# elfi-dev/elfi

Measured on AMD Instinct MI355X. Metric: ABC distances/sec, higher is better.
Workload: dtype f64; 1 GPU; configs[1]: synthetic Gaussian summaries, 1000000 samples x 32 summaries per GPU per step, elfi.Distance('euclidean'), inputs resident in HBM; samples_per_gpu=1000000, summaries=32, layout=row-major (n,m) f64, batches_in_rotation=3, exchange=none (N = 1), exchange_every=8, world_size_seen=1

## Files before the change

### elfi_amd/csrc/distance.hip

```cpp
#include "common.hpp"
#include "tile_stream.hpp"
#include "internal.hpp"
#include "np_sum.hpp"

#pragma clang fp contract(off)

namespace elfihip {

constexpr int kMaxTileM = 299;
constexpr int kMaxK = 64;

__device__ __forceinline__ double cbrt_halley(double s) {
  if (!(s > 0.0) || !(s < __builtin_huge_val())) return s;
  int e;
  double mant = frexp(s, &e);
  int q = e / 3, r = e - 3 * q;
  if (r < 0) {
    r += 3;
    q -= 1;
  }
  mant = ldexp(mant, r);
  double y = (double)__builtin_exp2f(__builtin_log2f((float)mant) * (1.0f / 3.0f));
  const double y3 = y * y * y;
  y = y * ((y3 + 2.0 * mant) / (2.0 * y3 + mant));
// ... 144 lines not shown
#pragma unroll 4
      for (int j = 0; j < m; ++j) {
        const double xc = kCentered ? x(j) - xmu : x(j);
        const double yc = kCentered ? y(j) - o.ymu : y(j);
        uv += xc * (yc * a(j));
        uu += xc * (xc * a(j));
      }
      return clip02(1.0 - uv / sqrt(uu * o.ynorm));
    } else {
      double xmu = 0.0;
      if constexpr (kCentered) xmu = np_pairwise_bounded<2>(x, 0, m) / (double)m;
      auto cx = [&](int j) { return kCentered ? x(j) - xmu : x(j); };
      auto cy = [&](int j) { return kCentered ? y(j) - o.ymu : y(j); };
      double s0 = 0.0, s1 = 0.0, q0 = 0.0, q1 = 0.0;
      int j = 0;
#pragma unroll 4
      for (; j + 1 < m; j += 2) {
        const double x0 = cx(j), x1 = cx(j + 1);
        s0 += x0 * cy(j);
        s1 += x1 * cy(j + 1);
        q0 += x0 * x0;
        q1 += x1 * x1;
      }
      double s = s0 + s1, q = q0 + q1;
      if (m & 1) {
        const double xl = cx(m - 1);
        s += xl * cy(m - 1);
        q += xl * xl;
      }
      return cos_finish(s, sqrt(q), o.ynorm);
    }
  }

  __device__ static __forceinline__ double cos_finish(double dot, double nx, double ny) {
    double c = dot / (nx * ny);
    if (fabs(c) > 1.0) c = copysign(1.0, c);
    return 1.0 - c;
  }
  __device__ static __forceinline__ double clip02(double d) { return d < 0.0 ? 0.0 : (d > 2.0 ? 2.0 : d); }

  __device__ static __forceinline__ double wide(const double* __restrict__ x, const double* __restrict__ y,
                                                const double* __restrict__ w, int m, int lane, const Obs& o) {
    auto wsum = [](double v) {
#pragma unroll
      for (int off = 32; off > 0; off >>= 1) v += __shfl_xor(v, off, 64);
      return v;
    };
    auto wn = [&](int j) { return kNormW ? w[j] / o.sw : (W ? w[j] : 1.0); };
    if constexpr (METRIC == ELFIHIP_CANBERRA || METRIC == ELFIHIP_BRAYCURTIS) {
      double s0 = 0.0, s1 = 0.0;
      for (int j = lane; j < m; j += 64) {
        const double xj = x[j], yj = y[j];
        if constexpr (METRIC == ELFIHIP_CANBERRA) {
          double num = fabs(xj - yj);
          const double den = fabs(xj) + fabs(yj);
          if constexpr (W) num = w[j] * num;
          s0 += num / (den + (den == 0.0 ? 1.0 : 0.0));
        } else {
          double dn = fabs(xj - yj), dd = fabs(xj + yj);
          if constexpr (W) {
            dn = w[j] * dn;
            dd = w[j] * dd;
          }
          s0 += dn;
          s1 += dd;
        }
      }
      s0 = wsum(s0);
      if constexpr (METRIC == ELFIHIP_CANBERRA) return s0;
      return s0 / wsum(s1);
    } else {
      double xmu = 0.0;
      if constexpr (kCentered) {
        for (int j = lane; j < m; j += 64) xmu += W ? x[j] * wn(j) : x[j];
        xmu = wsum(xmu);
        if constexpr (!W) xmu = xmu / (double)m;
      }
      double uv = 0.0, uu = 0.0;
      for (int j = lane; j < m; j += 64) {
        const double xc = x[j] - xmu, yc = y[j] - o.ymu;
        if constexpr (W) {
          uv += xc * (yc * wn(j));
          uu += xc * (xc * wn(j));
        } else {
          uv += xc * yc;
          uu += xc * xc;
        }
      }
      uv = wsum(uv);
      uu = wsum(uu);
      if constexpr (W) return clip02(1.0 - uv / sqrt(uu * o.ynorm));
      return cos_finish(uv, sqrt(uu), o.ynorm);
    }
  }
};

template <int METRIC, bool W>
__device__ __forceinline__ double kept_aux(double w, const Obs& o) {
  if constexpr (kRowMetric<METRIC> && Row<METRIC, W>::kNormW) return w / o.sw;
  return w;
}

template <int METRIC, bool W>
__device__ __forceinline__ Obs obs_of(const double* __restrict__ y, const double* __restrict__ aux, int m) {
  if constexpr (kRowMetric<METRIC>)
    return Row<METRIC, W>::obs([&](int j) { return y[j]; }, [&](int j) { return W ? aux[j] : 1.0; }, m);
  return Obs{1.0, 0.0, 0.0};
}

template <int METRIC, bool W, int U>
__global__ __launch_bounds__(256) void dist_rows_pipe_kernel(RowArgs A) {
  extern __shared__ __align__(16) double lds[];
  const int T = blockDim.x, tid = threadIdx.x, m = A.m;
  double* tile = lds;
  const int R = A.R;
  double* ys = tile + (size_t)R * A.mp;
  double* as = ys + m;
  const Obs o = obs_of<METRIC, W>(A.y, A.aux, m);
  for (int j = tid; j < m; j += T) {
    ys[j] = A.y[j];
    if constexpr (W) as[j] = kept_aux<METRIC, W>(A.aux[j], o);
  }
  const int64_t ntiles = (A.n + R - 1) / R;
  const double thr = A.F.thr ? *A.F.thr : 0.0;
  double2 v[U];
  int64_t t = blockIdx.x;
  if (t < ntiles) tile_fetch<U>(A, t * R, (int)((A.n - t * R) < R ? (A.n - t * R) : R), v);
  for (; t < ntiles; t += gridDim.x) {
    const int64_t row0 = t * R;
    const int rows = (int)((A.n - row0) < R ? (A.n - row0) : R);
    __syncthreads();
    tile_commit<U>(A, tile, rows, v);
    const int64_t tn = t + gridDim.x;
    if (tn < ntiles) tile_fetch<U>(A, tn * R, (int)((A.n - tn * R) < R ? (A.n - tn * R) : R), v);
    __syncthreads();
    double dist = 0.0;
    if (tid < rows) {
      const double* row = tile + (size_t)tid * A.mp;
      if constexpr (kRowMetric<METRIC>) {
        dist = Row<METRIC, W>::dist([&](int j) { return row[j]; }, [&](int j) { return ys[j]; },
                                    [&](int j) { return as[j]; }, m, o);
      } else {
        double s = Op<METRIC, W>::init();
#pragma unroll 8
        for (int j = 0; j < m; ++j) s = Op<METRIC, W>::step(s, row[j], ys[j], W ? as[j] : 1.0, A.p);
        dist = Op<METRIC, W>::finish(s, A.inv_p);
      }
      A.out[row0 + tid] = dist;
    }
    if (A.F.thr) reject_offer(A.F, tid < rows && dist < thr, dist, A.F.row_base + row0 + tid);
  }
}

template <int METRIC, bool W, int MM, int ROWS, int D, bool MERGE>
__global__ __launch_bounds__(64) void dist_rows_dma_kernel(RowArgs A) {
  extern __shared__ __align__(16) double lds[];
  constexpr int SLOT = ROWS * MM;
  constexpr int H = MM / 2;
  constexpr int PIECES = ROWS * H / 64;
  static_assert(ROWS <= 64 && (ROWS * H) % 64 == 0, "a slot is a whole number of 1 KiB DMA pieces, one row per lane");
  static_assert(D * SLOT * 8 >= REJ_FUSED_LDS, "the merge role works in the slot ring");
  if constexpr (MERGE) {
    if (blockIdx.x == 0) {
      reject_merge_wave(A.M, lds);
      return;
    }
  }
  const int lane = threadIdx.x;
  double* ring = lds;
  double* ys = lds + (size_t)D * SLOT;
  double* as = ys + MM;
  const unsigned lds_base = __builtin_amdgcn_readfirstlane((unsigned)(uintptr_t)ring);
  const Obs o = obs_of<METRIC, W>(A.y, A.aux, MM);
  if (lane < MM) {
    ys[lane] = A.y[lane];
    if constexpr (W) as[lane] = kept_aux<METRIC, W>(A.aux[lane], o);
  }
  const int64_t nslots = (A.n + ROWS - 1) / ROWS;
  const int64_t stride = MERGE ? gridDim.x - 1 : gridDim.x;
  double thr = 0.0;
  if (A.F.thr) {
    if constexpr (MERGE)
      thr = __hip_atomic_load(A.F.thr, __ATOMIC_RELAXED, __HIP_MEMORY_SCOPE_AGENT);
    else
      thr = *A.F.thr;
  }
  unsigned off[PIECES];
#pragma unroll
  for (int i = 0; i < PIECES; ++i) {
    const int G = i * 64 + lane;
    const int row = G / H, g = G % H;
    off[i] = (unsigned)(((int64_t)row * A.ldx + 2 * (g ^ dma_swizzle_key<MM>(row))) * 8);
  }
  asm volatile("s_waitcnt vmcnt(0) lgkmcnt(0)" ::: "memory");
  int64_t t = MERGE ? blockIdx.x - 1 : blockIdx.x;
#pragma unroll
  for (int k = 0; k < D - 1; ++k) {
    const int64_t tk = t + k * stride;
    if (tk < nslots) dma_issue_slot<MM, ROWS>(A, off, tk * ROWS, lds_base + (unsigned)(k * SLOT * 8), lane);
  }
  int cur = 0;
  for (; t < nslots; t += stride) {
    const int64_t tn = t + (int64_t)(D - 1) * stride;
    int nxt = cur + D - 1;
    if (nxt >= D) nxt -= D;
    if (tn < nslots) {
      dma_issue_slot<MM, ROWS>(A, off, tn * ROWS, lds_base + (unsigned)(nxt * SLOT * 8), lane);
      wait_vmcnt<PIECES * (D - 1)>();
    } else {
      wait_vmcnt<0>();
    }
    const int64_t row0 = t * ROWS;
    double dist = 0.0;
    const bool mine = (ROWS == 64 || lane < ROWS) && row0 + lane < A.n;
    if (ROWS == 64 || lane < ROWS) {
      const double* row = ring + (size_t)cur * SLOT + (size_t)lane * MM;
      const int key = dma_swizzle_key<MM>(lane);
      if constexpr (kRowMetric<METRIC>) {
        dist = Row<METRIC, W>::dist([&](int j) { return row[2 * ((j >> 1) ^ key) + (j & 1)]; },
                                    [&](int j) { return ys[j]; }, [&](int j) { return as[j]; }, MM, o);
      } else {
        double s = Op<METRIC, W>::init();
#pragma unroll
        for (int c = 0; c < H; ++c) {
          const double2 v = *reinterpret_cast<const double2*>(row + 2 * (c ^ key));
          const double2 yv = *reinterpret_cast<const double2*>(ys + 2 * c);
          double2 av = make_double2(1.0, 1.0);
          if constexpr (W) av = *reinterpret_cast<const double2*>(as + 2 * c);
          s = Op<METRIC, W>::step(s, v.x, yv.x, av.x, A.p);
          s = Op<METRIC, W>::step(s, v.y, yv.y, av.y, A.p);
        }
        dist = Op<METRIC, W>::finish(s, A.inv_p);
      }
      if (mine) A.out[row0 + lane] = dist;
    }
    if (A.F.thr) reject_offer(A.F, mine && dist < thr, dist, A.F.row_base + row0 + lane);
    asm volatile("s_waitcnt lgkmcnt(0)" ::: "memory");
    cur = cur + 1 == D ? 0 : cur + 1;
  }
}

template <int U>
__global__ __launch_bounds__(256) void dist_multiw_pipe_kernel(RowArgs A) {
  extern __shared__ __align__(16) double lds[];
  const int T = blockDim.x, tid = threadIdx.x, m = A.m, K = A.K;
  double* tile = lds;
  const int R = A.R;
  double* ys = tile + (size_t)R * A.mp;
  double* ws = ys + m;
  for (int j = tid; j < m; j += T) ys[j] = A.y[j];
  for (int j = tid; j < K * m; j += T) ws[j] = A.aux[j];
  const int64_t ntiles = (A.n + R - 1) / R;
  const double thr = A.F.thr ? *A.F.thr : 0.0;
  double2 v[U];
  int64_t t = blockIdx.x;
  if (t < ntiles) tile_fetch<U>(A, t * R, (int)((A.n - t * R) < R ? (A.n - t * R) : R), v);
  for (; t < ntiles; t += gridDim.x) {
    const int64_t row0 = t * R;
    const int rows = (int)((A.n - row0) < R ? (A.n - row0) : R);
    __syncthreads();
    tile_commit<U>(A, tile, rows, v);
    const int64_t tn = t + gridDim.x;
    if (tn < ntiles) tile_fetch<U>(A, tn * R, (int)((A.n - tn * R) < R ? (A.n - tn * R) : R), v);
    __syncthreads();
    double dlast = 0.0;
    if (tid < rows) {
      const double* row = tile + (size_t)tid * A.mp;
      for (int k0 = 0; k0 < K; k0 += 4) {
        const int kn = K - k0 < 4 ? K - k0 : 4;
        const double* w0 = ws + (size_t)k0 * m;
        const double* w1 = ws + (size_t)(k0 + (kn > 1 ? 1 : 0)) * m;
        const double* w2 = ws + (size_t)(k0 + (kn > 2 ? 2 : 0)) * m;
        const double* w3 = ws + (size_t)(k0 + (kn > 3 ? 3 : 0)) * m;
        double s0 = 0.0, s1 = 0.0, s2 = 0.0, s3 = 0.0;
#pragma unroll 4
        for (int j = 0; j < m; ++j) {
          const double d = row[j] - ys[j];
          const double d2 = d * d;
          s0 = s0 + w0[j] * d2;
          s1 = s1 + w1[j] * d2;
          s2 = s2 + w2[j] * d2;
          s3 = s3 + w3[j] * d2;
        }
        double* o = A.out + (row0 + tid) * K + k0;
        const double r0 = sqrt(s0), r1 = sqrt(s1), r2 = sqrt(s2), r3 = sqrt(s3);
        o[0] = r0;
        if (kn > 1) o[1] = r1;
        if (kn > 2) o[2] = r2;
        if (kn > 3) o[3] = r3;
        dlast = kn > 3 ? r3 : (kn > 2 ? r2 : (kn > 1 ? r1 : r0));
      }
    }
    if (A.F.thr) reject_offer(A.F, tid < rows && dlast < thr, dlast, A.F.row_base + row0 + tid);
  }
}

template <int METRIC, bool W, int U>
__global__ void dist_rows_kernel(RowArgs A) {
  extern __shared__ __align__(16) double lds[];
  const int T = blockDim.x, tid = threadIdx.x, m = A.m;
  double* tile = lds;
  double* ys = tile + (size_t)T * A.mp;
  double* as = ys + m;
  const Obs o = obs_of<METRIC, W>(A.y, A.aux, m);
  for (int j = tid; j < m; j += T) {
    ys[j] = A.y[j];
    if constexpr (W) as[j] = kept_aux<METRIC, W>(A.aux[j], o);
  }
  const int64_t ntiles = (A.n + T - 1) / T;
  for (int64_t t = blockIdx.x; t < ntiles; t += gridDim.x) {
    const int64_t row0 = t * T;
    const int rows = (int)((A.n - row0) < T ? (A.n - row0) : T);
    __syncthreads();
    load_tile<U>(A, tile, row0, rows);
    __syncthreads();
    if (tid < rows) {
      const double* row = tile + (size_t)tid * A.mp;
      if constexpr (kRowMetric<METRIC>) {
        A.out[row0 + tid] = Row<METRIC, W>::dist([&](int j) { return row[j]; }, [&](int j) { return ys[j]; },
                                                 [&](int j) { return as[j]; }, m, o);
      } else {
        double s = Op<METRIC, W>::init();
#pragma unroll 4
        for (int j = 0; j < m; ++j) s = Op<METRIC, W>::step(s, row[j], ys[j], W ? as[j] : 1.0, A.p);
        A.out[row0 + tid] = Op<METRIC, W>::finish(s, A.inv_p);
      }
    }
  }
}

template <int U>
__global__ void dist_rows_mahalanobis_kernel(RowArgs A) {
  extern __shared__ __align__(16) double lds[];
  const int T = blockDim.x, tid = threadIdx.x, m = A.m;
  double* tile = lds;
  double* ys = tile + (size_t)T * A.mp;
  for (int j = tid; j < m; j += T) ys[j] = A.y[j];
  const double* __restrict__ VI = A.aux;
  const int64_t ntiles = (A.n + T - 1) / T;
  for (int64_t t = blockIdx.x; t < ntiles; t += gridDim.x) {
    const int64_t row0 = t * T;
    const int rows = (int)((A.n - row0) < T ? (A.n - row0) : T);
    __syncthreads();
    load_tile<U>(A, tile, row0, rows);
    __syncthreads();
    if (tid < rows) {
      double* row = tile + (size_t)tid * A.mp;
      for (int j = 0; j < m; ++j) row[j] = row[j] - ys[j];
      double s = 0.0;
      for (int i = 0; i < m; ++i) {
        double ti = 0.0;
        const double* vi = VI + (size_t)i * m;
        for (int k = 0; k < m; ++k) ti += row[k] * vi[k];
        s += row[i] * ti;
      }
      A.out[row0 + tid] = sqrt(s);
    }
  }
}

constexpr int MAHA_ROWS = 64;
typedef double v4d __attribute__((ext_vector_type(4)));

__global__ __launch_bounds__(256) void dist_rows_mahalanobis_mfma_kernel(RowArgs A) {
  extern __shared__ __align__(16) double lds[];
  const int tid = threadIdx.x, l = tid & 63, w = tid >> 6, m = A.m;
  const int mk = (m + 3) & ~3, mc = (m + 15) & ~15;
  const int dp = mc | 1;
  double* dl = lds;
  double* vi = dl + MAHA_ROWS * dp;
  for (int e = tid; e < mk * mc; e += 256) {
    const int k = e / mc, c = e - k * mc;
    vi[e] = (k < m && c < m) ? A.aux[(size_t)k * m + c] : 0.0;
  }
  const int64_t ntiles = (A.n + MAHA_ROWS - 1) / MAHA_ROWS;
  for (int64_t t = blockIdx.x; t < ntiles; t += gridDim.x) {
    const int64_t row0 = t * MAHA_ROWS;
    const int rows = (int)((A.n - row0) < MAHA_ROWS ? (A.n - row0) : MAHA_ROWS);
    __syncthreads();
    for (int e = tid; e < MAHA_ROWS * dp; e += 256) {
      const int r = e / dp, c = e - r * dp;
      dl[e] = (r < rows && c < m) ? A.X[(row0 + r) * A.ldx + c] - A.y[c] : 0.0;
    }
    __syncthreads();
    const double* da = dl + (16 * w + (l & 15)) * dp + (l >> 4);
    double part[4] = {0.0, 0.0, 0.0, 0.0};
    for (int ct0 = 0; ct0 < mc / 16; ct0 += 4) {
      v4d acc[4];
#pragma unroll
      for (int j = 0; j < 4; ++j) acc[j] = (v4d){0.0, 0.0, 0.0, 0.0};
      for (int s_ = 0; s_ < mk / 4; ++s_) {
// ... 223 lines not shown
    x[2 * h + 1] = t.y;
  }
}

template <int METRIC, bool W, int M, int U>
__global__ __launch_bounds__(256) void dist_rows_narrow_kernel(RowArgs A) {
  const int tid = threadIdx.x;
  double yv[M], av[M];
  const Obs o = obs_of<METRIC, W>(A.y, A.aux, M);
#pragma unroll
  for (int j = 0; j < M; ++j) {
    yv[j] = A.y[j];
    av[j] = W ? kept_aux<METRIC, W>(A.aux[j], o) : 1.0;
  }
  const double thr = A.F.thr ? *A.F.thr : 0.0;
  const int64_t per = 256 * U;
  for (int64_t base = (int64_t)blockIdx.x * per; base < A.n; base += (int64_t)gridDim.x * per) {
    double x[U][M];
#pragma unroll
    for (int u = 0; u < U; ++u) {
      const int64_t r = base + u * 256 + tid;
      narrow_load<M>(A, r < A.n ? r : A.n - 1, x[u]);
    }
#pragma unroll
    for (int u = 0; u < U; ++u) {
      const int64_t r = base + u * 256 + tid;
      double dist;
      if constexpr (kRowMetric<METRIC>) {
        dist = Row<METRIC, W>::dist([&](int j) { return x[u][j]; }, [&](int j) { return yv[j]; },
                                    [&](int j) { return av[j]; }, M, o);
      } else {
        double s = Op<METRIC, W>::init();
#pragma unroll
        for (int j = 0; j < M; ++j) s = Op<METRIC, W>::step(s, x[u][j], yv[j], av[j], A.p);
        dist = Op<METRIC, W>::finish(s, A.inv_p);
      }
      if (r < A.n) A.out[r] = dist;
      if (A.F.thr) reject_offer(A.F, r < A.n && dist < thr, dist, A.F.row_base + r);
    }
  }
}

template <int M, int U>
__global__ __launch_bounds__(256) void dist_rows_mahalanobis_narrow_kernel(RowArgs A) {
  const int tid = threadIdx.x;
  double yv[M], vi[M][M];
#pragma unroll
  for (int j = 0; j < M; ++j) {
    yv[j] = A.y[j];
#pragma unroll
    for (int k = 0; k < M; ++k) vi[j][k] = A.aux[j * M + k];
  }
  const int64_t per = 256 * U;
  for (int64_t base = (int64_t)blockIdx.x * per; base < A.n; base += (int64_t)gridDim.x * per) {
    double x[U][M];
#pragma unroll
    for (int u = 0; u < U; ++u) {
      const int64_t r = base + u * 256 + tid;
      narrow_load<M>(A, r < A.n ? r : A.n - 1, x[u]);
    }
#pragma unroll
    for (int u = 0; u < U; ++u) {
      const int64_t r = base + u * 256 + tid;
      double d[M];
#pragma unroll
      for (int j = 0; j < M; ++j) d[j] = x[u][j] - yv[j];
      double s = 0.0;
#pragma unroll
      for (int i = 0; i < M; ++i) {
        double ti = 0.0;
#pragma unroll
        for (int k = 0; k < M; ++k) ti += d[k] * vi[i][k];
        s += d[i] * ti;
      }
      if (r < A.n) A.out[r] = sqrt(s);
    }
  }
}

template <int M, int U>
__global__ __launch_bounds__(256) void dist_multiw_narrow_kernel(RowArgs A) {
  constexpr int KMAX = 8;
  __shared__ __align__(16) double stage_all[4 * 64 * KMAX];
  const int tid = threadIdx.x, K = A.K;
  double* stage = stage_all + (tid >> 6) * 64 * KMAX;
  const bool staged = (reinterpret_cast<uintptr_t>(A.out) & 15u) == 0;
  double yv[M], wv[KMAX][M];
#pragma unroll
  for (int j = 0; j < M; ++j) yv[j] = A.y[j];
#pragma unroll
  for (int k = 0; k < KMAX; ++k)
#pragma unroll
    for (int j = 0; j < M; ++j) wv[k][j] = k < K ? A.aux[k * M + j] : 0.0;
  const double thr = A.F.thr ? *A.F.thr : 0.0;
  const int64_t per = 256 * U;
  for (int64_t base = (int64_t)blockIdx.x * per; base < A.n; base += (int64_t)gridDim.x * per) {
    double x[U][M];
#pragma unroll
    for (int u = 0; u < U; ++u) {
      const int64_t r = base + u * 256 + tid;
      narrow_load<M>(A, r < A.n ? r : A.n - 1, x[u]);
    }
#pragma unroll
    for (int u = 0; u < U; ++u) {
      const int64_t r = base + u * 256 + tid;
      double d2[M];
#pragma unroll
      for (int j = 0; j < M; ++j) {
        const double d = x[u][j] - yv[j];
        d2[j] = d * d;
      }
      double dlast = 0.0, dk[KMAX];
#pragma unroll
      for (int k = 0; k < KMAX; ++k) {
        dk[k] = 0.0;
        if (k < K) {
          double sk = 0.0;
#pragma unroll
          for (int j = 0; j < M; ++j) sk = sk + wv[k][j] * d2[j];
          dlast = sqrt(sk);
          dk[k] = dlast;
          if (!staged && r < A.n) A.out[r * K + k] = dlast;
        }
      }
      if (staged) {
        const int64_t r0 = base + u * 256 + (tid & ~63);
        const int64_t left = A.n - r0;
        if (left > 0) wave_store_rows<KMAX>(stage, A.out + r0 * K, dk, K, tid & 63, left < 64 ? (int)left : 64);
      }
      if (A.F.thr) reject_offer(A.F, r < A.n && dlast < thr, dlast, A.F.row_base + r);
    }
  }
}

static inline bool narrow_rows(const elfihip_ctx* ctx, const RowArgs& A) {
  return A.vec2 && (A.m == 2 || A.m == 4) && ctx->dist_form != 1;
}
static inline unsigned narrow_grid(const elfihip_ctx* ctx, int64_t n, int U) {
  int64_t g = (n + 256 * U - 1) / (256 * U), cap = (int64_t)ctx->cu_count * 8;
  if (g > cap) g = cap;
  return (unsigned)(g < 1 ? 1 : g);
}

static int pipe_unroll(int m, bool light) {
  if (!light) return m <= 16 ? 8 : 16;
  return m <= 32 ? 4 : (m <= 64 ? 8 : 16);
}

template <int METRIC, bool W>
constexpr bool kDma16 = METRIC != ELFIHIP_CANBERRA;
template <int METRIC, bool W>
constexpr bool kDma64 = !(METRIC == ELFIHIP_CANBERRA || (METRIC == ELFIHIP_CORRELATION && W));

template <int METRIC, bool W>
static int launch_rows(elfihip_ctx* ctx, RowArgs A, bool* filtered, bool* merged) {
  if (A.m > kMaxTileM) {
    int64_t rows_per_block = 4;
    int64_t g = (A.n + rows_per_block - 1) / rows_per_block;
    int64_t cap = (int64_t)ctx->cu_count * 8;
    if (g > cap) g = cap;
    hipLaunchKernelGGL((dist_rows_wide_kernel<METRIC, W>), dim3((unsigned)g), dim3(256), 0, ctx->stream, A);
    return launch_status(ctx, "dist_rows_wide_kernel");
  }
  if (narrow_rows(ctx, A)) {
    constexpr int U = 4;
    if (A.m == 2)
      hipLaunchKernelGGL((dist_rows_narrow_kernel<METRIC, W, 2, U>), dim3(narrow_grid(ctx, A.n, U)), dim3(256), 0, ctx->stream, A);
    else
      hipLaunchKernelGGL((dist_rows_narrow_kernel<METRIC, W, 4, U>), dim3(narrow_grid(ctx, A.n, U)), dim3(256), 0, ctx->stream, A);
    if (filtered) *filtered = A.F.thr != nullptr;
    return launch_status(ctx, "dist_rows_narrow_kernel");
  }
  size_t lds;
  const int T = pick_block(A.m, 2 * (size_t)A.m, &lds);
  const int64_t ntiles = (A.n + T - 1) / T;
  const int g = grid_for(ctx, ntiles, lds, T);
  if (A.vec2 && ctx->dist_form != 1 && METRIC != ELFIHIP_MINKOWSKI && METRIC != ELFIHIP_SEUCLIDEAN &&
      ((A.m == 16 && kDma16<METRIC, W>) || A.m == 32 || (A.m == 64 && kDma64<METRIC, W>)) && A.ldx <= (1 << 21)) {
    const int rows = A.m == 64 ? 32 : 64;
    const int D = A.m == 16 ? 4 : 2;
    const size_t ldsd = ((size_t)D * rows * A.m + 2 * (size_t)A.m) * sizeof(double);
    const bool merge = A.M.k > 0 && A.F.thr != nullptr;
    int64_t gd = (int64_t)ctx->cu_count * 4;
    const int64_t nslots = (A.n + rows - 1) / rows;
    if (gd > nslots + (merge ? 1 : 0)) gd = nslots + (merge ? 1 : 0);
    if (gd < 1) gd = 1;
    const dim3 grid((unsigned)gd), block(64);
    if (merge) {
      if (A.m == 16) {
        if constexpr (kDma16<METRIC, W>)
          hipLaunchKernelGGL((dist_rows_dma_kernel<METRIC, W, 16, 64, 4, true>), grid, block, ldsd, ctx->stream, A);
      } else if (A.m == 32)
        hipLaunchKernelGGL((dist_rows_dma_kernel<METRIC, W, 32, 64, 2, true>), grid, block, ldsd, ctx->stream, A);
      else if constexpr (kDma64<METRIC, W>)
        hipLaunchKernelGGL((dist_rows_dma_kernel<METRIC, W, 64, 32, 2, true>), grid, block, ldsd, ctx->stream, A);
      if (merged) *merged = true;
    } else if (A.m == 16) {
      if constexpr (kDma16<METRIC, W>)
        hipLaunchKernelGGL((dist_rows_dma_kernel<METRIC, W, 16, 64, 4, false>), grid, block, ldsd, ctx->stream, A);
    } else if (A.m == 32) {
      hipLaunchKernelGGL((dist_rows_dma_kernel<METRIC, W, 32, 64, 2, false>), grid, block, ldsd, ctx->stream, A);
    } else if constexpr (kDma64<METRIC, W>) {
      hipLaunchKernelGGL((dist_rows_dma_kernel<METRIC, W, 64, 32, 2, false>), grid, block, ldsd, ctx->stream, A);
    }
    if (filtered) *filtered = A.F.thr != nullptr;
    return launch_status(ctx, "dist_rows_dma_kernel");
  }
  if (A.vec2 && A.m <= 128) {
    const int Tp = 128, U = pipe_unroll(A.m, METRIC != ELFIHIP_MINKOWSKI);
    int R = 2 * Tp * U / A.m;
    if (R > Tp) R = Tp;
    A.R = R;
    const size_t ldsp = ((size_t)R * A.mp + 2 * (size_t)A.m) * sizeof(double);
    const int gp = grid_for(ctx, (A.n + R - 1) / R, ldsp, Tp);
    if (U == 4)
      hipLaunchKernelGGL((dist_rows_pipe_kernel<METRIC, W, 4>), dim3(gp), dim3(Tp), ldsp, ctx->stream, A);
    else if (U == 8)
      hipLaunchKernelGGL((dist_rows_pipe_kernel<METRIC, W, 8>), dim3(gp), dim3(Tp), ldsp, ctx->stream, A);
    else
      hipLaunchKernelGGL((dist_rows_pipe_kernel<METRIC, W, 16>), dim3(gp), dim3(Tp), ldsp, ctx->stream, A);
    if (filtered) *filtered = A.F.thr != nullptr;
    return launch_status(ctx, "dist_rows_pipe_kernel");
  }
  if (T == 64) {
    ELFIHIP_TRY(set_lds(ctx, dist_rows_kernel<METRIC, W, 16>, lds));
    hipLaunchKernelGGL((dist_rows_kernel<METRIC, W, 16>), dim3(g), dim3(T), lds, ctx->stream, A);
  } else {
    hipLaunchKernelGGL((dist_rows_kernel<METRIC, W, 8>), dim3(g), dim3(T), lds, ctx->stream, A);
  }
  return launch_status(ctx, "dist_rows_kernel");
}

template <int METRIC, bool W>
static int launch_cols(elfihip_ctx* ctx, ColArgs A) {
  const int T = 256;
  int64_t work = (A.vec2 && !kRowMetric<METRIC>) ? ((A.n + 1) >> 1) : A.n;
  int64_t g = (work + T - 1) / T;
  int64_t cap = (int64_t)ctx->cu_count * 8;
  if (g > cap) g = cap;
  if (g < 1) g = 1;
  size_t lds = 2 * (size_t)A.m * sizeof(double);
  hipLaunchKernelGGL((dist_cols_kernel<METRIC, W>), dim3((unsigned)g), dim3(T), lds, ctx->stream, A);
  return launch_status(ctx, "dist_cols_kernel");
}

static int canonical_metric(elfihip_ctx* ctx, int metric, double p, const double* aux, int* out_metric) {
  switch (metric) {
    case ELFIHIP_EUCLIDEAN:
    case ELFIHIP_SQEUCLIDEAN:
    case ELFIHIP_CITYBLOCK:
    case ELFIHIP_CHEBYSHEV:
      *out_metric = metric;
      return ELFIHIP_OK;
    case ELFIHIP_MINKOWSKI:
      if (!(p > 0.0)) return fail(ctx, ELFIHIP_ERR_ARG, "minkowski needs p > 0 (got %g)", p);
      if (p == 1.0)
        *out_metric = ELFIHIP_CITYBLOCK;
      else if (p == 2.0)
        *out_metric = ELFIHIP_EUCLIDEAN;
      else if (p > 1.7e308)
        *out_metric = ELFIHIP_CHEBYSHEV;
      else
        *out_metric = ELFIHIP_MINKOWSKI;
      return ELFIHIP_OK;
    case ELFIHIP_SEUCLIDEAN:
      if (!aux) return fail(ctx, ELFIHIP_ERR_ARG, "seuclidean needs V");
      *out_metric = metric;
      return ELFIHIP_OK;
    case ELFIHIP_MAHALANOBIS:
      if (!aux) return fail(ctx, ELFIHIP_ERR_ARG, "mahalanobis needs VI");
      *out_metric = metric;
      return ELFIHIP_OK;
    case ELFIHIP_CANBERRA:
    case ELFIHIP_BRAYCURTIS:
    case ELFIHIP_COSINE:
    case ELFIHIP_CORRELATION:
      *out_metric = metric;
      return ELFIHIP_OK;
    default:
      return fail(ctx, ELFIHIP_ERR_ARG, "unknown metric id %d", metric);
  }
}

static bool aligned16(const void* p) { return (reinterpret_cast<uintptr_t>(p) & 15u) == 0; }

static RowArgs make_row_args(const double* dX, int64_t n, int m, int64_t ldx, const double* dy,
                             const double* daux, double p, double* dout) {
  RowArgs A;
  A.X = dX;
  A.n = n;
  A.ldx = ldx;
  A.y = dy;
  A.aux = daux;
  A.out = dout;
  A.p = p;
  A.inv_p = p != 0.0 ? 1.0 / p : 0.0;
  A.m = m;
  A.mp = m | 1;
  A.K = 0;
  A.R = 0;
  A.nt = 0;
  A.F = RejectFilter{nullptr, nullptr, nullptr, nullptr, 0u, 0ll};
  A.M = RejectMergeJob{};
  A.vec2 = (m % 2 == 0) && (ldx % 2 == 0) && aligned16(dX);
  A.div_h = make_fastdiv((uint32_t)(A.vec2 ? m / 2 : m));
  return A;
}

template <int KC>
__global__ __launch_bounds__(256, 2) void dist_rows_mahalanobis_reg_kernel(RowArgs A) {
  extern __shared__ __align__(16) double lds[];
  constexpr int U = 8;
  const int tid = threadIdx.x, l = tid & 63, w = tid >> 6, m = A.m, mp = A.mp;
  double* tile = lds;
  double* ys = tile + MAHA_ROWS * mp + 64;
  for (int e = tid; e < 64; e += 256) tile[MAHA_ROWS * mp + e] = 0.0;
  for (int e = tid; e < 16 * KC; e += 256) ys[e] = e < m ? A.y[e] : 0.0;
  double b[4 * KC][KC], yc[KC];
#pragma unroll
  for (int s_ = 0; s_ < 4 * KC; ++s_) {
    const int k = 4 * s_ + (l >> 4);
#pragma unroll
    for (int j = 0; j < KC; ++j) {
      const int c = 16 * j + (l & 15);
      b[s_][j] = (k < m && c < m) ? A.aux[(size_t)k * m + c] : 0.0;
    }
  }
#pragma unroll
  for (int j = 0; j < KC; ++j) yc[j] = (16 * j + (l & 15)) < m ? A.y[16 * j + (l & 15)] : 0.0;
  const int64_t ntiles = (A.n + MAHA_ROWS - 1) / MAHA_ROWS;
  double2 v[U];
  int64_t t = blockIdx.x;
  if (t < ntiles) tile_fetch<U>(A, t * MAHA_ROWS, (int)((A.n - t * MAHA_ROWS) < MAHA_ROWS ? (A.n - t * MAHA_ROWS) : MAHA_ROWS), v);
  for (; t < ntiles; t += gridDim.x) {
    const int64_t row0 = t * MAHA_ROWS;
    const int rows = (int)((A.n - row0) < MAHA_ROWS ? (A.n - row0) : MAHA_ROWS);
    __syncthreads();
    tile_commit<U>(A, tile, rows, v);
    const int64_t tn = t + gridDim.x;
    if (tn < ntiles) tile_fetch<U>(A, tn * MAHA_ROWS, (int)((A.n - tn * MAHA_ROWS) < MAHA_ROWS ? (A.n - tn * MAHA_ROWS) : MAHA_ROWS), v);
    __syncthreads();
    const double* xa = tile + (16 * w + (l & 15)) * mp + (l >> 4);
    double part[4] = {0.0, 0.0, 0.0, 0.0};
#pragma unroll
    for (int j = 0; j < KC; ++j) {
      v4d acc = (v4d){0.0, 0.0, 0.0, 0.0};
#pragma unroll
      for (int s_ = 0; s_ < 4 * KC; ++s_) {
        const int k = 4 * s_ + (l >> 4);
        const double a = k < m ? xa[4 * s_] - ys[k] : 0.0;
        acc = __builtin_amdgcn_mfma_f64_16x16x4f64(a, b[s_][j], acc, 0, 0, 0);
      }
      const int c = 16 * j + (l & 15);
#pragma unroll
      for (int i = 0; i < 4; ++i) {
        const double dlt = c < m ? tile[(16 * w + (l >> 4) + 4 * i) * mp + c] - yc[j] : 0.0;
        part[i] += acc[i] * dlt;
      }
    }
// ... 395 lines not shown
```

### elfi_amd/csrc/tile_stream.hpp

```cpp
#pragma once

#include "common.hpp"

namespace elfihip {

struct FastDiv {
  uint32_t mul, d;
};
static inline FastDiv make_fastdiv(uint32_t d) {
  FastDiv f;
  f.d = d;
  uint64_t q = (1ull << 32) / d;
  f.mul = q > 0xFFFFFFFFull ? 0xFFFFFFFFu : (uint32_t)q;
  return f;
}
__device__ __forceinline__ uint32_t fastdiv(uint32_t x, FastDiv f) {
  uint32_t q = __umulhi(x, f.mul);
  if (x - q * f.d >= f.d) ++q;
  return q;
}

struct RejectFilter {
  const double* thr;
  double* cval;
// ... 86 lines not shown
      }
    }
  } else {
    const uint32_t m = (uint32_t)A.m;
    const uint32_t nel = (uint32_t)rows * m;
    for (uint32_t base = 0; base < nel; base += (uint32_t)(T * U)) {
      double v[U];
      uint32_t r[U], j[U];
#pragma unroll
      for (int u = 0; u < U; ++u) {
        uint32_t idx = base + (uint32_t)(u * T + tid);
        bool ok = idx < nel;
        uint32_t q = fastdiv(ok ? idx : 0u, A.div_h);
        r[u] = q;
        j[u] = (ok ? idx : 0u) - q * m;
        if (ok) v[u] = X[(int64_t)q * A.ldx + j[u]];
      }
#pragma unroll
      for (int u = 0; u < U; ++u) {
        uint32_t idx = base + (uint32_t)(u * T + tid);
        if (idx < nel) tile[r[u] * (uint32_t)A.mp + j[u]] = v[u];
      }
    }
  }
}

template <int U>
__device__ __forceinline__ void tile_fetch(const RowArgs& A, int64_t row0, int rows, double2 (&v)[U]) {
  const int T = blockDim.x, tid = threadIdx.x;
  const double* __restrict__ X = A.X + row0 * A.ldx;
  const uint32_t h = (uint32_t)A.m >> 1;
  const uint32_t npairs = (uint32_t)rows * h;
#pragma unroll
  for (int u = 0; u < U; ++u) {
    const uint32_t idx = (uint32_t)(u * T + tid);
    const bool ok = idx < npairs;
    const uint32_t q = fastdiv(ok ? idx : 0u, A.div_h);
    const uint32_t jj = (ok ? idx : 0u) - q * h;
    v[u] = make_double2(0.0, 0.0);
    if (ok) {
      const double2* src = reinterpret_cast<const double2*>(X + (int64_t)q * A.ldx + 2 * jj);
      if (A.nt) {
        typedef double v2d_nt __attribute__((ext_vector_type(2)));
        const v2d_nt t = __builtin_nontemporal_load(reinterpret_cast<const v2d_nt*>(src));
        v[u] = make_double2(t.x, t.y);
      } else {
        v[u] = *src;
      }
    }
  }
}

template <int U>
__device__ __forceinline__ void tile_commit(const RowArgs& A, double* tile, int rows, const double2 (&v)[U]) {
  const int T = blockDim.x, tid = threadIdx.x;
  const uint32_t h = (uint32_t)A.m >> 1;
  const uint32_t npairs = (uint32_t)rows * h;
#pragma unroll
  for (int u = 0; u < U; ++u) {
    const uint32_t idx = (uint32_t)(u * T + tid);
    if (idx < npairs) {
      const uint32_t q = fastdiv(idx, A.div_h);
      const uint32_t jj = idx - q * h;
      double* dst = tile + q * (uint32_t)A.mp + 2 * jj;
      dst[0] = v[u].x;
      dst[1] = v[u].y;
    }
  }
}


#if defined(__HIPCC__)
template <bool NT>
__device__ __forceinline__ void dma16_to_lds(const void* gsrc, unsigned lds_dst) {
  unsigned keep;
  if constexpr (NT)
    asm volatile("s_mov_b32 %0, m0\n\ts_mov_b32 m0, %2\n\ts_nop 0\n\tglobal_load_lds_dwordx4 %1, off nt\n\ts_mov_b32 m0, %0"
                 : "=&s"(keep) : "v"(gsrc), "s"(lds_dst) : "memory");
  else
    asm volatile("s_mov_b32 %0, m0\n\ts_mov_b32 m0, %2\n\ts_nop 0\n\tglobal_load_lds_dwordx4 %1, off\n\ts_mov_b32 m0, %0"
                 : "=&s"(keep) : "v"(gsrc), "s"(lds_dst) : "memory");
}
template <int N>
__device__ __forceinline__ void wait_vmcnt() {
  asm volatile("s_waitcnt vmcnt(%0)" ::"i"(N) : "memory");
}
template <int MM>
__device__ __forceinline__ int dma_swizzle_key(int row) {
  constexpr int H = MM / 2;
  constexpr int RP = H >= 16 ? 1 : 16 / H;
  constexpr int MASK = (H >= 16 ? 16 : H) - 1;
  return (row / RP) & MASK;
}
template <bool NT>
__device__ __forceinline__ void dma16_to_lds_off(const void* base, unsigned voff, unsigned lds_dst) {
  unsigned keep;
  if constexpr (NT)
    asm volatile("s_mov_b32 %0, m0\n\ts_mov_b32 m0, %3\n\ts_nop 0\n\tglobal_load_lds_dwordx4 %1, %2 nt\n\ts_mov_b32 m0, %0"
                 : "=&s"(keep) : "v"(voff), "s"(base), "s"(lds_dst) : "memory");
  else
    asm volatile("s_mov_b32 %0, m0\n\ts_mov_b32 m0, %3\n\ts_nop 0\n\tglobal_load_lds_dwordx4 %1, %2\n\ts_mov_b32 m0, %0"
                 : "=&s"(keep) : "v"(voff), "s"(base), "s"(lds_dst) : "memory");
}
template <int MM, int ROWS>
__device__ __forceinline__ void dma_issue_slot(const RowArgs& A, const unsigned (&off)[ROWS * (MM / 2) / 64], int64_t row0,
                                               unsigned lds_slot, int lane) {
  constexpr int H = MM / 2;
  constexpr int PIECES = ROWS * H / 64;
  if (row0 + ROWS <= A.n) {
    const uint64_t p = (uint64_t)(A.X + row0 * A.ldx);
    const uint64_t b = (uint64_t)(unsigned)__builtin_amdgcn_readfirstlane((unsigned)p) |
                       ((uint64_t)(unsigned)__builtin_amdgcn_readfirstlane((unsigned)(p >> 32)) << 32);
#pragma unroll
    for (int i = 0; i < PIECES; ++i) dma16_to_lds_off<true>((const void*)b, off[i], lds_slot + (unsigned)i * 1024u);
  } else {
#pragma unroll
    for (int i = 0; i < PIECES; ++i) {
      const int G = i * 64 + lane;
      const int row = G / H, g = G % H;
      int64_t gr = row0 + row;
      if (gr >= A.n) gr = A.n - 1;
      dma16_to_lds<true>(A.X + gr * A.ldx + 2 * (g ^ dma_swizzle_key<MM>(row)), lds_slot + (unsigned)i * 1024u);
    }
  }
}

template <int KMAX>
__device__ __forceinline__ void wave_store_rows(double* stage, double* dst, const double (&vals)[KMAX], int K, int lane, int nv) {
  typedef double v2d_st __attribute__((ext_vector_type(2)));
#pragma unroll
  for (int k = 0; k < KMAX; ++k)
    if (k < K) stage[lane * K + k] = vals[k];
  asm volatile("s_waitcnt lgkmcnt(0)" ::: "memory");
  __builtin_amdgcn_wave_barrier();
  const int total = nv * K, npieces = total >> 1;
#pragma unroll
  for (int i = 0; i < (KMAX + 1) / 2; ++i) {
    const int p = lane + 64 * i;
    if (p < npieces) *reinterpret_cast<v2d_st*>(dst + 2 * p) = *reinterpret_cast<const v2d_st*>(stage + 2 * p);
  }
  if ((total & 1) && lane == 0) dst[total - 1] = stage[total - 1];
  asm volatile("s_waitcnt lgkmcnt(0)" ::: "memory");
  __builtin_amdgcn_wave_barrier();
}

struct __attribute__((aligned(16))) RejEnt {
  double v;
  long long r;
};
__device__ __forceinline__ bool rej_before(const RejEnt& a, const RejEnt& b) {
  return a.v < b.v || (a.v == b.v && a.r < b.r);
}

__device__ __forceinline__ void reject_merge_wave(const RejectMergeJob& J, void* smem) {
  RejEnt* st = reinterpret_cast<RejEnt*>(smem);
  RejEnt* ch = st + REJ_FUSED_MAX_K;
  const int lane = threadIdx.x, k = J.k;
  const double inf = __longlong_as_double(0x7ff0000000000000ll);
  const long long maxrow = 0x7fffffffffffffffll;
  unsigned int c = *J.count;
  if (c > J.cap) {
    if (lane == 0) atomicOr(J.status, 1u);
    c = J.cap;
  }
  constexpr int PER = REJ_FUSED_CHUNK / 64;
  static_assert(REJ_FUSED_MAX_K / 64 == PER, "one register set for the state's and the chunks' loads");
  double lv[PER];
  long long lr[PER];
#pragma unroll
  for (int u = 0; u < PER; ++u) {
    const int e = min(lane + 64 * u, k - 1);
    lv[u] = J.best_val[e];
    lr[u] = J.best_row[e];
  }
#pragma unroll
  for (int u = 0; u < PER; ++u)
    if (lane + 64 * u < k) st[lane + 64 * u] = RejEnt{lv[u], lr[u]};
  for (unsigned int c0 = 0; c0 < c; c0 += REJ_FUSED_CHUNK) {
    const int nc = (int)min((unsigned int)REJ_FUSED_CHUNK, c - c0);
    int P = 64;
    while (P < nc) P <<= 1;
    int nv = 0;
#pragma unroll
    for (int u = 0; u < PER; ++u) {
      const unsigned int idx = c0 + (unsigned int)min(lane + 64 * u, nc - 1);
      lv[u] = J.cand_val[idx];
      lr[u] = J.cand_row[idx];
    }
#pragma unroll
    for (int u = 0; u < PER; ++u) {
      const int i = lane + 64 * u;
      const bool ok = i < nc && lv[u] == lv[u];
      nv += __popcll(__ballot(ok));
      if (i < P) ch[i] = ok ? RejEnt{lv[u], lr[u]} : RejEnt{inf, maxrow};
    }
    __syncthreads();
    for (int size = 2; size <= P; size <<= 1)
      for (int stride = size >> 1; stride > 0; stride >>= 1) {
        double av[PER / 2], bv[PER / 2];
        long long ar[PER / 2], br[PER / 2];
#pragma unroll
        for (int u = 0; u < PER / 2; ++u) {
          const int q = lane + 64 * u;
          const int i = 2 * (q & (P / 2 - 1)) - (q & (stride - 1));
          const RejEnt x = ch[i], y = ch[i + stride];
          av[u] = x.v;
          ar[u] = x.r;
          bv[u] = y.v;
          br[u] = y.r;
        }
#pragma unroll
        for (int u = 0; u < PER / 2; ++u) {
          const int q = lane + 64 * u;
          if (q < P / 2) {
            const int i = 2 * q - (q & (stride - 1));
            const bool asc = (i & size) == 0;
            if (rej_before(RejEnt{bv[u], br[u]}, RejEnt{av[u], ar[u]}) == asc) {
              ch[i] = RejEnt{bv[u], br[u]};
              ch[i + stride] = RejEnt{av[u], ar[u]};
            }
          }
        }
        __syncthreads();
      }
    constexpr int QMAX = REJ_FUSED_MAX_K / 64;
    const int Q = (k + 63) / 64;
    const int d0 = min(lane * Q, k), d1 = min(d0 + Q, k);
    int lo = max(0, d0 - nv), hi = min(d0, k);
    while (lo < hi) {
      const int mid = (lo + hi) >> 1;
      if (rej_before(st[mid], ch[d0 - 1 - mid]))
        lo = mid + 1;
      else
        hi = mid;
    }
    double ov[QMAX];
    long long orow[QMAX];
    int ia = lo, ib = d0 - lo;
#pragma unroll
    for (int q = 0; q < QMAX; ++q) {
      ov[q] = 0.0;
      orow[q] = 0;
      if (d0 + q < d1) {
        const RejEnt sa = st[ia < k ? ia : k - 1], cb = ch[ib < nv ? ib : 0];
        const bool take_state = ib >= nv || (ia < k && rej_before(sa, cb));
        ov[q] = take_state ? sa.v : cb.v;
        orow[q] = take_state ? sa.r : cb.r;
        ia += take_state ? 1 : 0;
        ib += take_state ? 0 : 1;
      }
    }
    __syncthreads();
#pragma unroll
    for (int q = 0; q < QMAX; ++q)
      if (d0 + q < d1) st[d0 + q] = RejEnt{ov[q], orow[q]};
    __syncthreads();
  }
  __syncthreads();
#pragma unroll
  for (int u = 0; u < PER; ++u) {
    const RejEnt x = st[min(lane + 64 * u, k - 1)];
    lv[u] = x.v;
    lr[u] = x.r;
  }
  const double kth = st[k - 1].v;
#pragma unroll
  for (int u = 0; u < PER; ++u) {
    const int e = lane + 64 * u;
    if (e < k) {
      J.best_val[e] = lv[u];
      J.best_row[e] = lr[u];
    }
  }
  if (J.export_val) {
#pragma unroll
    for (int u = 0; u < PER; ++u) {
      const int e = lane + 64 * u;
      if (e < k) {
        J.export_val[e] = lv[u];
        reinterpret_cast<long long*>(J.export_val + k)[e] = lr[u];
      }
    }
  }
  if (lane == 0) {
    *J.thr = kth;
    *J.count = 0u;
  }
}

#endif

static inline bool tile_aligned16(const void* p) { return (reinterpret_cast<uintptr_t>(p) & 15u) == 0; }

}
```

Before: 23.22 billion distances/s.

## Replace single-wave DMA kernel with producer/consumer LDS ring per workgroup

The one-wave-per-block DMA distance kernel becomes a persistent kernel with one workgroup per CU. One loader wave keeps several slots of DMA loads in flight into a large LDS ring, and several consumer waves compute distances, coordinating through full/freed flags in LDS. The merge role now runs as a separate wave inside block 0 instead of taking a whole block, and its block-wide barriers become wave-local syncs. Output is written with relaxed atomic stores. The goal is to decouple load latency from compute and keep HBM streaming continuously, at the cost of spin-wait handshakes, one block per CU, and more complex synchronisation.

```diff
diff --git a/elfi_amd/csrc/distance.hip b/elfi_amd/csrc/distance.hip
--- a/elfi_amd/csrc/distance.hip
+++ b/elfi_amd/csrc/distance.hip
@@ -320,32 +320,103 @@
   }
 }
 
-template <int METRIC, bool W, int MM, int ROWS, int D, bool MERGE>
-__global__ __launch_bounds__(64) void dist_rows_dma_kernel(RowArgs A) {
+template <int METRIC, bool W>
+constexpr int kRingConsumers = kRowMetric<METRIC> ? 7 : 3;
+
+template <int P, int K>
+__device__ __forceinline__ void wait_slots(int rem) {
+  if constexpr (K > 1) {
+    if (rem >= K - 1) {
+      wait_vmcnt<P * (K - 1)>();
+      return;
+    }
+    wait_slots<P, K - 1>(rem);
+  } else {
+    wait_vmcnt<0>();
+  }
+}
+
+__device__ __forceinline__ void store_wt_f64(double* p, double v) {
+  typedef __attribute__((address_space(1))) unsigned long long gu64;
+  __hip_atomic_store((gu64*)(p), (unsigned long long)__double_as_longlong(v), __ATOMIC_RELAXED, __HIP_MEMORY_SCOPE_AGENT);
+}
+
+template <int MM, int C, bool MERGE>
+struct RingGeom {
+  static constexpr int ROWS = MM == 64 ? 32 : 64;
+  static constexpr int SLOT = ROWS * MM;
+  static constexpr int PIECES = ROWS * (MM / 2) / 64;
+  static constexpr int F = MM == 16 ? 6 : 3;
+  static constexpr int S = F + 4;
+  static constexpr int MERGE_D = MERGE ? REJ_FUSED_LDS / 8 : 0;
+  static constexpr size_t lds_bytes() { return ((size_t)S * SLOT + MERGE_D + (size_t)C * 2 * MM) * 8 + (size_t)2 * S * 4; }
+  static_assert(F * PIECES < 64, "the loader's counted waits cover every slot it keeps in flight");
+};
+
+template <int METRIC, bool W, int MM, int C, bool MERGE>
+__global__ __launch_bounds__(64 * (C + 2)) void dist_rows_ring_kernel(RowArgs A) {
   extern __shared__ __align__(16) double lds[];
-  constexpr int SLOT = ROWS * MM;
+  using Gm = RingGeom<MM, C, MERGE>;
+  constexpr int ROWS = Gm::ROWS, SLOT = Gm::SLOT, PIECES = Gm::PIECES, F = Gm::F, S = Gm::S;
   constexpr int H = MM / 2;
-  constexpr int PIECES = ROWS * H / 64;
   static_assert(ROWS <= 64 && (ROWS * H) % 64 == 0, "a slot is a whole number of 1 KiB DMA pieces, one row per lane");
-  static_assert(D * SLOT * 8 >= REJ_FUSED_LDS, "the merge role works in the slot ring");
-  if constexpr (MERGE) {
-    if (blockIdx.x == 0) {
-      reject_merge_wave(A.M, lds);
-      return;
-    }
-  }
-  const int lane = threadIdx.x;
+  const int lane = threadIdx.x & 63, wave = threadIdx.x >> 6;
   double* ring = lds;
-  double* ys = lds + (size_t)D * SLOT;
+  volatile unsigned* full = reinterpret_cast<volatile unsigned*>(lds + (size_t)S * SLOT + Gm::MERGE_D + (size_t)C * 2 * MM);
+  volatile unsigned* freed = full + S;
+  const int64_t G = gridDim.x;
+  const int64_t nslots = (A.n + ROWS - 1) / ROWS;
+  const int nloc = (int)((nslots - blockIdx.x + G - 1) / G);
+
+  if (wave == 0) {
+    const unsigned lds_base = __builtin_amdgcn_readfirstlane((unsigned)(uintptr_t)ring);
+    unsigned off[PIECES];
+#pragma unroll
+    for (int i = 0; i < PIECES; ++i) {
+      const int Gi = i * 64 + lane;
+      const int row = Gi / H, g = Gi % H;
+      off[i] = (unsigned)(((int64_t)row * A.ldx + 2 * (g ^ dma_swizzle_key<MM>(row))) * 8);
+    }
+#pragma unroll
+    for (int k = 0; k < F; ++k)
+      if (k < nloc)
+        dma_issue_slot<MM, ROWS>(A, off, (blockIdx.x + k * G) * ROWS, lds_base + (unsigned)(k * SLOT * 8), lane);
+    if (lane < S) {
+      full[lane] = 0u;
+      freed[lane] = 0u;
+    }
+    asm volatile("s_waitcnt lgkmcnt(0)" ::: "memory");
+    __builtin_amdgcn_s_barrier();
+    int pub = 0, nxt = F % S;
+    for (int i = 0; i < nloc; ++i) {
+      const int rem = nloc - 1 - i;
+      wait_slots<PIECES, F>(rem < F - 1 ? rem : F - 1);
+      full[pub] = (unsigned)(i + 1);
+      pub = pub + 1 == S ? 0 : pub + 1;
+      const int j = i + F;
+      if (j < nloc) {
+        if (j >= S)
+          while (freed[nxt] < (unsigned)(j - S + 1)) __builtin_amdgcn_s_sleep(1);
+        dma_issue_slot<MM, ROWS>(A, off, (blockIdx.x + (int64_t)j * G) * ROWS, lds_base + (unsigned)(nxt * SLOT * 8), lane);
+        nxt = nxt + 1 == S ? 0 : nxt + 1;
+      }
+    }
+    return;
+  }
+  if (wave > C) {
+    __builtin_amdgcn_s_barrier();
+    if constexpr (MERGE)
+      if (blockIdx.x == 0) reject_merge_wave(A.M, lds + (size_t)S * SLOT);
+    return;
+  }
+  const int c = wave - 1;
+  double* ys = lds + (size_t)S * SLOT + Gm::MERGE_D + (size_t)c * 2 * MM;
   double* as = ys + MM;
-  const unsigned lds_base = __builtin_amdgcn_readfirstlane((unsigned)(uintptr_t)ring);
   const Obs o = obs_of<METRIC, W>(A.y, A.aux, MM);
   if (lane < MM) {
     ys[lane] = A.y[lane];
     if constexpr (W) as[lane] = kept_aux<METRIC, W>(A.aux[lane], o);
   }
-  const int64_t nslots = (A.n + ROWS - 1) / ROWS;
-  const int64_t stride = MERGE ? gridDim.x - 1 : gridDim.x;
   double thr = 0.0;
   if (A.F.thr) {
     if constexpr (MERGE)
@@ -353,58 +424,47 @@
     else
       thr = *A.F.thr;
   }
-  unsigned off[PIECES];
-#pragma unroll
-  for (int i = 0; i < PIECES; ++i) {
-    const int G = i * 64 + lane;
-    const int row = G / H, g = G % H;
-    off[i] = (unsigned)(((int64_t)row * A.ldx + 2 * (g ^ dma_swizzle_key<MM>(row))) * 8);
-  }
-  asm volatile("s_waitcnt vmcnt(0) lgkmcnt(0)" ::: "memory");
-  int64_t t = MERGE ? blockIdx.x - 1 : blockIdx.x;
-#pragma unroll
-  for (int k = 0; k < D - 1; ++k) {
-    const int64_t tk = t + k * stride;
-    if (tk < nslots) dma_issue_slot<MM, ROWS>(A, off, tk * ROWS, lds_base + (unsigned)(k * SLOT * 8), lane);
-  }
-  int cur = 0;
-  for (; t < nslots; t += stride) {
-    const int64_t tn = t + (int64_t)(D - 1) * stride;
-    int nxt = cur + D - 1;
-    if (nxt >= D) nxt -= D;
-    if (tn < nslots) {
-      dma_issue_slot<MM, ROWS>(A, off, tn * ROWS, lds_base + (unsigned)(nxt * SLOT * 8), lane);
-      wait_vmcnt<PIECES * (D - 1)>();
-    } else {
-      wait_vmcnt<0>();
-    }
-    const int64_t row0 = t * ROWS;
+  __builtin_amdgcn_s_barrier();
+  const int key = dma_swizzle_key<MM>(lane);
+  int pos = c;
+  for (int i = c; i < nloc; i += C) {
+    while (full[pos] != (unsigned)(i + 1)) __builtin_amdgcn_s_sleep(1);
+    asm volatile("" ::: "memory");
+    const int64_t row0 = (blockIdx.x + (int64_t)i * G) * ROWS;
+    const double* row = ring + (size_t)pos * SLOT + (size_t)lane * MM;
     double dist = 0.0;
     const bool mine = (ROWS == 64 || lane < ROWS) && row0 + lane < A.n;
-    if (ROWS == 64 || lane < ROWS) {
-      const double* row = ring + (size_t)cur * SLOT + (size_t)lane * MM;
-      const int key = dma_swizzle_key<MM>(lane);
-      if constexpr (kRowMetric<METRIC>) {
+    if constexpr (kRowMetric<METRIC>) {
+      if (ROWS == 64 || lane < ROWS)
         dist = Row<METRIC, W>::dist([&](int j) { return row[2 * ((j >> 1) ^ key) + (j & 1)]; },
                                     [&](int j) { return ys[j]; }, [&](int j) { return as[j]; }, MM, o);
-      } else {
+      asm volatile("s_waitcnt lgkmcnt(0)" ::: "memory");
+      freed[pos] = (unsigned)(i + 1);
+    } else {
+      double2 v[H];
+      if (ROWS == 64 || lane < ROWS) {
+#pragma unroll
+        for (int q = 0; q < H; ++q) v[q] = *reinterpret_cast<const double2*>(row + 2 * (q ^ key));
+      }
+      asm volatile("s_waitcnt lgkmcnt(0)" ::: "memory");
+      freed[pos] = (unsigned)(i + 1);
+      if (ROWS == 64 || lane < ROWS) {
         double s = Op<METRIC, W>::init();
 #pragma unroll
-        for (int c = 0; c < H; ++c) {
-          const double2 v = *reinterpret_cast<const double2*>(row + 2 * (c ^ key));
-          const double2 yv = *reinterpret_cast<const double2*>(ys + 2 * c);
+        for (int q = 0; q < H; ++q) {
+          const double2 yv = *reinterpret_cast<const double2*>(ys + 2 * q);
           double2 av = make_double2(1.0, 1.0);
-          if constexpr (W) av = *reinterpret_cast<const double2*>(as + 2 * c);
-          s = Op<METRIC, W>::step(s, v.x, yv.x, av.x, A.p);
-          s = Op<METRIC, W>::step(s, v.y, yv.y, av.y, A.p);
+          if constexpr (W) av = *reinterpret_cast<const double2*>(as + 2 * q);
+          s = Op<METRIC, W>::step(s, v[q].x, yv.x, av.x, A.p);
+          s = Op<METRIC, W>::step(s, v[q].y, yv.y, av.y, A.p);
         }
         dist = Op<METRIC, W>::finish(s, A.inv_p);
       }
-      if (mine) A.out[row0 + lane] = dist;
-    }
+    }
+    if (mine) store_wt_f64(A.out + row0 + lane, dist);
     if (A.F.thr) reject_offer(A.F, mine && dist < thr, dist, A.F.row_base + row0 + lane);
-    asm volatile("s_waitcnt lgkmcnt(0)" ::: "memory");
-    cur = cur + 1 == D ? 0 : cur + 1;
+    pos += C;
+    if (pos >= S) pos -= S;
   }
 }
 
@@ -934,6 +994,25 @@
 template <int METRIC, bool W>
 constexpr bool kDma64 = !(METRIC == ELFIHIP_CANBERRA || (METRIC == ELFIHIP_CORRELATION && W));
 
+template <int METRIC, bool W, int MM, bool MERGE>
+static int launch_ring(elfihip_ctx* ctx, const RowArgs& A, int64_t nslots) {
+  constexpr int C = kRingConsumers<METRIC, W>;
+  constexpr size_t lds = RingGeom<MM, C, MERGE>::lds_bytes();
+  static_assert(lds > 80 * 1024 && lds <= 160 * 1024, "one workgroup per CU: more than half of the CU's 160 KiB of LDS");
+  static unsigned raised = 0;
+  const unsigned bit = 1u << (ctx->device & 31);
+  if (!(raised & bit)) {
+    ELFIHIP_TRY(set_lds(ctx, dist_rows_ring_kernel<METRIC, W, MM, C, MERGE>, lds));
+    raised |= bit;
+  }
+  int64_t g = ctx->cu_count;
+  if (g > nslots) g = nslots;
+  if (g < 1) g = 1;
+  hipLaunchKernelGGL((dist_rows_ring_kernel<METRIC, W, MM, C, MERGE>), dim3((unsigned)g), dim3(64 * (C + 1 + (MERGE ? 1 : 0))),
+                     lds, ctx->stream, A);
+  return launch_status(ctx, "dist_rows_ring_kernel");
+}
+
 template <int METRIC, bool W>
 static int launch_rows(elfihip_ctx* ctx, RowArgs A, bool* filtered, bool* merged) {
   if (A.m > kMaxTileM) {
@@ -959,34 +1038,27 @@
   const int g = grid_for(ctx, ntiles, lds, T);
   if (A.vec2 && ctx->dist_form != 1 && METRIC != ELFIHIP_MINKOWSKI && METRIC != ELFIHIP_SEUCLIDEAN &&
       ((A.m == 16 && kDma16<METRIC, W>) || A.m == 32 || (A.m == 64 && kDma64<METRIC, W>)) && A.ldx <= (1 << 21)) {
-    const int rows = A.m == 64 ? 32 : 64;
-    const int D = A.m == 16 ? 4 : 2;
-    const size_t ldsd = ((size_t)D * rows * A.m + 2 * (size_t)A.m) * sizeof(double);
     const bool merge = A.M.k > 0 && A.F.thr != nullptr;
-    int64_t gd = (int64_t)ctx->cu_count * 4;
-    const int64_t nslots = (A.n + rows - 1) / rows;
-    if (gd > nslots + (merge ? 1 : 0)) gd = nslots + (merge ? 1 : 0);
-    if (gd < 1) gd = 1;
-    const dim3 grid((unsigned)gd), block(64);
+    const int64_t nslots = (A.n + (A.m == 64 ? 32 : 64) - 1) / (A.m == 64 ? 32 : 64);
+    int rc = ELFIHIP_OK;
     if (merge) {
       if (A.m == 16) {
-        if constexpr (kDma16<METRIC, W>)
-          hipLaunchKernelGGL((dist_rows_dma_kernel<METRIC, W, 16, 64, 4, true>), grid, block, ldsd, ctx->stream, A);
-      } else if (A.m == 32)
-        hipLaunchKernelGGL((dist_rows_dma_kernel<METRIC, W, 32, 64, 2, true>), grid, block, ldsd, ctx->stream, A);
-      else if constexpr (kDma64<METRIC, W>)
-        hipLaunchKernelGGL((dist_rows_dma_kernel<METRIC, W, 64, 32, 2, true>), grid, block, ldsd, ctx->stream, A);
+        if constexpr (kDma16<METRIC, W>) rc = launch_ring<METRIC, W, 16, true>(ctx, A, nslots);
+      } else if (A.m == 32) {
+        rc = launch_ring<METRIC, W, 32, true>(ctx, A, nslots);
+      } else if constexpr (kDma64<METRIC, W>) {
+        rc = launch_ring<METRIC, W, 64, true>(ctx, A, nslots);
+      }
       if (merged) *merged = true;
     } else if (A.m == 16) {
-      if constexpr (kDma16<METRIC, W>)
-        hipLaunchKernelGGL((dist_rows_dma_kernel<METRIC, W, 16, 64, 4, false>), grid, block, ldsd, ctx->stream, A);
+      if constexpr (kDma16<METRIC, W>) rc = launch_ring<METRIC, W, 16, false>(ctx, A, nslots);
     } else if (A.m == 32) {
-      hipLaunchKernelGGL((dist_rows_dma_kernel<METRIC, W, 32, 64, 2, false>), grid, block, ldsd, ctx->stream, A);
+      rc = launch_ring<METRIC, W, 32, false>(ctx, A, nslots);
     } else if constexpr (kDma64<METRIC, W>) {
-      hipLaunchKernelGGL((dist_rows_dma_kernel<METRIC, W, 64, 32, 2, false>), grid, block, ldsd, ctx->stream, A);
+      rc = launch_ring<METRIC, W, 64, false>(ctx, A, nslots);
     }
     if (filtered) *filtered = A.F.thr != nullptr;
-    return launch_status(ctx, "dist_rows_dma_kernel");
+    return rc;
   }
   if (A.vec2 && A.m <= 128) {
     const int Tp = 128, U = pipe_unroll(A.m, METRIC != ELFIHIP_MINKOWSKI);
diff --git a/elfi_amd/csrc/tile_stream.hpp b/elfi_amd/csrc/tile_stream.hpp
--- a/elfi_amd/csrc/tile_stream.hpp
+++ b/elfi_amd/csrc/tile_stream.hpp
@@ -262,10 +262,15 @@
   return a.v < b.v || (a.v == b.v && a.r < b.r);
 }
 
+__device__ __forceinline__ void wave_lds_sync() {
+  asm volatile("s_waitcnt lgkmcnt(0)" ::: "memory");
+  __builtin_amdgcn_wave_barrier();
+}
+
 __device__ __forceinline__ void reject_merge_wave(const RejectMergeJob& J, void* smem) {
   RejEnt* st = reinterpret_cast<RejEnt*>(smem);
   RejEnt* ch = st + REJ_FUSED_MAX_K;
-  const int lane = threadIdx.x, k = J.k;
+  const int lane = threadIdx.x & 63, k = J.k;
   const double inf = __longlong_as_double(0x7ff0000000000000ll);
   const long long maxrow = 0x7fffffffffffffffll;
   unsigned int c = *J.count;
@@ -304,7 +309,7 @@
       nv += __popcll(__ballot(ok));
       if (i < P) ch[i] = ok ? RejEnt{lv[u], lr[u]} : RejEnt{inf, maxrow};
     }
-    __syncthreads();
+    wave_lds_sync();
     for (int size = 2; size <= P; size <<= 1)
       for (int stride = size >> 1; stride > 0; stride >>= 1) {
         double av[PER / 2], bv[PER / 2];
@@ -331,7 +336,7 @@
             }
           }
         }
-        __syncthreads();
+        wave_lds_sync();
       }
     constexpr int QMAX = REJ_FUSED_MAX_K / 64;
     const int Q = (k + 63) / 64;
@@ -360,13 +365,13 @@
         ib += take_state ? 0 : 1;
       }
     }
-    __syncthreads();
+    wave_lds_sync();
 #pragma unroll
     for (int q = 0; q < QMAX; ++q)
       if (d0 + q < d1) st[d0 + q] = RejEnt{ov[q], orow[q]};
-    __syncthreads();
-  }
-  __syncthreads();
+    wave_lds_sync();
+  }
+  wave_lds_sync();
 #pragma unroll
   for (int u = 0; u < PER; ++u) {
     const RejEnt x = st[min(lane + 64 * u, k - 1)];
```

Result: slower. 16.74 billion distances/s (median of 2 runs) (-27.9%).
